# astomodynamics/cddp-cpp

Hardware: AMD Instinct MI355X
Metric: trajectories_per_sec (higher is better)
Workload: dtype f64

## Files before the change

### cddp-cpp_amd/csrc/capi.hip

```cpp
#include <algorithm>
#include <chrono>
#include <cmath>
#include <cstdarg>
#include <cstddef>
#include <cstdio>
#include <cstdlib>
#include <cstring>
#include <string>
#include <vector>
#include <map>

#include "launch.hpp"
#include "plant.hpp"
#include "io_kernels.hpp"
#include "sens_kernels.hpp"
#include "score_kernels.hpp"
#include "mppi_kernels.hpp"

static int ladder_strictly_decreasing(const double *a, int n) {
  for (int i = 1; i < n; ++i) if (!(a[i] < a[i - 1])) return 0;
  return n > 0 ? 1 : 0;
}

using namespace cddp_dev;
// ... 850 lines not shown
  HIPCHK(hipStreamSynchronize(h->stream));
  return 0;
}

static int in_set_terminal(Inner *h, const double *S_T, const double *Y_T, const double *Lambda_T) {
  if (!h) return fail(-1, "null handle");
  if (h->P.n_term <= 0) return fail(-1, "cddp_hip_set_terminal: the problem has no terminal constraints");
  if (!h->has_state) return fail(-1, "cddp_hip_set_terminal needs an initialised handle");
  HIPCHK(hipSetDevice(h->device));
  const DevBuf &d = h->d;
  struct { const double *host; double *dev; int n; } items[] = {{S_T, d.ST, h->P.mT}, {Y_T, d.YT, h->P.mT}, {Lambda_T, d.LamT, h->P.pT}};
  for (auto &it : items) {
    if (!it.host || it.n <= 0) continue;
    std::vector<double> buf((size_t)it.n * d.Bp, 0.0);
    for (int b = 0; b < d.B; ++b) for (int i = 0; i < it.n; ++i) buf[(size_t)i * d.Bp + b] = it.host[(size_t)b * it.n + i];
    HIPCHK(hipMemcpyAsync(it.dev, buf.data(), buf.size() * sizeof(double), hipMemcpyHostToDevice, h->stream));
    HIPCHK(hipStreamSynchronize(h->stream));
  }
  return 0;
}

static int in_backward(Inner *h, int32_t *ok) {
  if (!h) return fail(-1, "null handle");
  HIPCHK(hipSetDevice(h->device));
  if (!h->initialized) { int rc = in_initialize(h); if (rc) return rc; }
  h->ks->derivs(h->d, h->route, 1, h->stream);
  h->ks->backward(h->d, h->route, h->P.solver, 1, 0, h->stream);
  HIPCHK(hipGetLastError());
  if (ok) HIPCHK(hipMemcpyAsync(ok, h->d.bwd_ok, sizeof(int) * h->d.B, hipMemcpyDeviceToHost, h->stream));
  HIPCHK(hipStreamSynchronize(h->stream));
  return 0;
}

static int in_forward(Inner *h, const double *alphas, int n_alphas, cddp_hip_trial *trials) {
  if (!h || !alphas || !trials) return fail(-1, "null argument");
  if (n_alphas <= 0 || n_alphas > h->d.n_alphas) return fail(-1, "n_alphas must be in [1, %d] (the handle's ladder size)", h->d.n_alphas);
  HIPCHK(hipSetDevice(h->device));
  ProblemDev tmp = h->P;
  for (int i = 0; i < n_alphas; ++i) tmp.alphas[i] = alphas[i];
  HIPCHK(hipMemcpyAsync(h->dP, &tmp, sizeof(ProblemDev), hipMemcpyHostToDevice, h->stream));
  DevBuf dcall = h->d;
  dcall.ladder_sorted = ladder_strictly_decreasing(tmp.alphas, h->d.n_alphas);
  h->ks->forward(dcall, h->route, h->P.solver, 0, n_alphas, PH_FWD1, 1, 0, h->stream, 0, 0);
  h->ks->costate(dcall, h->route, h->P.solver, 0, n_alphas, PH_FWD1, 1, 0, h->stream);
  HIPCHK(hipGetLastError());
  const DevBuf &d = h->d;
  const size_t n = (size_t)n_alphas * d.Bp;
  std::vector<double> c(n), mf(n), th(n), ipr(n), ic(n), ap(n), ad(n);
  std::vector<int> su(n);
  HIPCHK(hipMemcpyAsync(c.data(), d.t_cost, n * 8, hipMemcpyDeviceToHost, h->stream));
  HIPCHK(hipMemcpyAsync(mf.data(), d.t_merit, n * 8, hipMemcpyDeviceToHost, h->stream));
  HIPCHK(hipMemcpyAsync(th.data(), d.t_theta, n * 8, hipMemcpyDeviceToHost, h->stream));
  HIPCHK(hipMemcpyAsync(ipr.data(), d.t_inf_pr, n * 8, hipMemcpyDeviceToHost, h->stream));
  HIPCHK(hipMemcpyAsync(ic.data(), d.t_inf_comp, n * 8, hipMemcpyDeviceToHost, h->stream));
  HIPCHK(hipMemcpyAsync(ap.data(), d.t_apr, n * 8, hipMemcpyDeviceToHost, h->stream));
  HIPCHK(hipMemcpyAsync(ad.data(), d.t_adu, n * 8, hipMemcpyDeviceToHost, h->stream));
  HIPCHK(hipMemcpyAsync(su.data(), d.t_success, n * 4, hipMemcpyDeviceToHost, h->stream));
  HIPCHK(hipMemcpyAsync(h->dP, &h->P, sizeof(ProblemDev), hipMemcpyHostToDevice, h->stream));
  HIPCHK(hipStreamSynchronize(h->stream));
  for (int b = 0; b < d.B; ++b)
    for (int a = 0; a < n_alphas; ++a) {
      cddp_hip_trial &t = trials[(size_t)b * n_alphas + a];
      const size_t i = (size_t)a * d.Bp + b;
      t.alpha = alphas[a]; t.alpha_pr = ap[i]; t.alpha_du = ad[i]; t.cost = c[i]; t.merit_function = mf[i];
      t.theta = th[i]; t.inf_pr = ipr[i]; t.inf_comp = ic[i]; t.success = (su[i] == 1) ? 1 : 0; t._pad = 0;
    }
  return 0;
}

struct SolveRun {
  Inner *h = nullptr;
  bool want_stats = false;
  int conc = 1;
  int detail = -1;
  std::vector<int> ev_slot;
  size_t ev_used = 0;
// ... 28 lines not shown
    const bool want = detail == CDDP_HIP_TIMING_ALL ||
                      (detail == CDDP_HIP_TIMING_ROLLOUT && (point == 1 || point == 2 || (two_stage_marks && (point == 3 || point == 4)))) ||
                      (detail == CDDP_HIP_TIMING_SWEEP && (point == 0 || point == 1));
    if (!want) return;
    if (ev_used == h->ev_pool.size()) {
      hipEvent_t e;
      if ((h->knob->event_fence ? hipEventCreate(&e) : hipEventCreateWithFlags(&e, hipEventDisableSystemFence)) != hipSuccess) return;
      h->ev_pool.push_back(e);
    }
    const size_t slot = (size_t)6 * (size_t)(outer - 1) + (size_t)point;
    if (ev_slot.size() <= slot) ev_slot.resize(slot + 1, -1);
    hipEventRecord(h->ev_pool[ev_used], h->stream);
    ev_slot[slot] = (int)ev_used++;
  }

  void adapt_ladder(int window_iters) {
    if (pinned) return;
    long total = 0;
    std::vector<long> hd(na + 1);
    for (int a = 0; a <= na; ++a) { hd[a] = (long)hist_now[a] - (long)hist_prev[a]; total += hd[a]; }
    hist_prev = hist_now;
    if (total <= 0) return;
    const long allow = std::max(1L, (long)window_iters / 4);
    int kq = na;
    long tail = hd[na];
    for (int k = na - 1; k >= 1; --k) {
      tail += hd[k];
      if (tail <= allow) kq = k; else break;
    }
    if (kq >= na - 1) {
      if (waves_all <= 2048) { one_stage = true; }
      else { one_stage = false; k1 = k_cap2; }
    } else {
      one_stage = false; k1 = std::max(1, std::min(kq + h->knob->ls_margin, k_cap));
      if (waves_all <= 2048 && (long)k1 * per_alpha_waves > two_stage_max_waves) one_stage = true;
      const long small_cap = (h->P.solver == CDDP_HIP_SOLVER_LOGDDP || h->P.solver == CDDP_HIP_SOLVER_MSIPDDP) ? 2048 : 1024;
      if (waves_all <= small_cap && h->P.nx <= 8 && h->knob->ls_small_frac * k1 > na) one_stage = true;
    }
    if (h->knob->debug_ladder) {
      std::fprintf(stderr, "[ladder] it=%d total=%ld kq=%d -> %s k1=%d hist:", outer, total, kq, one_stage ? "one" : "two", k1);
      for (int a = 0; a <= na; ++a) std::fprintf(stderr, " %ld", hd[a]);
      std::fprintf(stderr, "\n");
    }
  }

  int begin(Inner *h_, bool stats_, int conc_) {
    h = h_; want_stats = stats_; conc = std::max(1, conc_);
    const ProblemDev &P = h->P;
    const DevBuf &d = h->d;
    hipStream_t s = h->stream;
    const KernelSet *ks = h->ks;
    max_it = P.opt.max_iterations;
    first_rule = (P.ls_rule == CDDP_HIP_LS_FIRST_SUCCESS);
    na = d.n_alphas;
    use_graph = h->knob->graph;
    if (use_graph && conc > 1) {
      static bool said = false;
      if (!said) { said = true; std::fprintf(stderr, "[cddp_hip] CDDP_HIP_GRAPH=1: graph replay does not keep the CU-masked streams' partition; the tile groups share the whole chip\n"); }
    }
    detail = (want_stats && !use_graph) ? h->timing_detail : -1;
    if (!h->ev_begin) { HIPCHK(hipEventCreate(&h->ev_begin)); HIPCHK(hipEventCreate(&h->ev_end)); }
    if (!h->ev_poll) { HIPCHK(hipEventCreateWithFlags(&h->ev_poll, hipEventDisableTiming)); HIPCHK(hipEventCreateWithFlags(&h->ev_poll2, hipEventDisableTiming)); }
    poll_evs[0] = h->ev_poll; poll_evs[1] = h->ev_poll2;
    win_enq = win_dig = 0; ran_ahead = false;
    if (!h->h_poll) HIPCHK(hipHostMalloc((void **)&h->h_poll, sizeof(int) * 2 * kPollWords));
    HIPCHK(hipMemsetAsync(h->d_launched, 0, sizeof(unsigned long long) * kLsGran, s));
    HIPCHK(hipEventRecord(h->ev_begin, s));
    pre_has_state = h->has_state;
    shadow = !force_sync && shadow_eligible(h, conc) && max_it > 0;
    redo_needed = false;
    inkernel = shadow && P.ls_rule == CDDP_HIP_LS_FIRST_SUCCESS && h->knob->ls_inkernel &&
               (h->route.rollout == Route::kPair || h->route.rollout == Route::kTwoConsumers);
    poll_us = h->knob->ls_poll_us >= 0 ? h->knob->ls_poll_us : kLsPollUs;
    h->ls_counts[0] = h->ls_counts[1] = h->ls_counts[2] = 0;
    if (inkernel && !h->h_ls) HIPCHK(hipHostMalloc((void **)&h->h_ls, sizeof(unsigned long long) * kLsGran));
    h->last_shadow = shadow; h->ever_solved = true;
    if (shadow) HIPCHK(hipMemsetAsync(h->d.cs_bad, 0, sizeof(int), s));
// ... 23 lines not shown
  void enqueue_iteration(int last) {
    const ProblemDev &P = h->P;
    if (shadow) {
      DevBuf &hd = h->d;
      hd.Vx_prev = hd.Vx; hd.Vxx_prev = hd.Vxx;
      std::swap(hd.Vx, hd.Vx2); std::swap(hd.Vxx, hd.Vxx2);
      hd.cs_vsel ^= 1;
    }
    DevBuf dsh = h->d;
    if (shadow) {
      h->cs_epoch += 2;
      dsh.cs_mode = 1; dsh.cs_stamp = h->cs_epoch + 1; dsh.cs_want = dsh.cs_stamp - 2;
      dsh.cs_fail_stamp = h->knob->fail_shadow > 0 ? stamp0 + 2 * h->knob->fail_shadow + 1 : 0;
    }
    const DevBuf &d = dsh;
    hipStream_t s = h->stream;
    const KernelSet *ks = h->ks;
    const Route &r = h->route;
    hipStream_t sf = h->cu.fwd ? h->cu.fwd : s;
    auto to_fwd = [&](int k) { if (sf != s) { order_check(hipEventRecord(h->cu.ev[k], s)); order_check(hipStreamWaitEvent(sf, h->cu.ev[k], 0)); } };
    auto from_fwd = [&](int k) { if (sf != s) { order_check(hipEventRecord(h->cu.ev[k], sf)); order_check(hipStreamWaitEvent(s, h->cu.ev[k], 0)); } };
    const bool split = !one_stage && inkernel;
    two_stage_marks = !one_stage && !split;
    mark(0);
    ks->derivs(d, r, 0, s);
    tl_sweep_hop = h->cu.sweep ? &h->cu.hop : nullptr;
    if (shadow && outer > 1) { dsh.cs_extra = ks->shadow_extra(d, r); ks->backward(dsh, r, P.solver, 0, 1, s); dsh.cs_extra = 0; }
    else ks->backward(d, r, P.solver, 0, 1, s);
    tl_sweep_hop = nullptr;
    mark(1);
    to_fwd(0);
    if (fwd_wait) hipStreamWaitEvent(sf, fwd_wait, 0);
    if (one_stage || split) {
      ks->forward(d, r, P.solver, 0, na, PH_FWD1, 0, first_rule ? 1 : 0, sf, split ? k1 : 0, poll_us);
      if (fwd_done) hipEventRecord(fwd_done, sf);
      from_fwd(1);
      mark(2);
      if (!shadow) ks->costate(d, r, P.solver, 0, na, PH_FWD1, 0, first_rule ? 1 : 2, s);
      ks->update(d, r, 1, na, last, 1, s);
      mark(3);
      launches += shadow ? 3 : 4;
    } else {
      ks->forward(d, r, P.solver, 0, k1, PH_FWD1, 0, 1, sf, 0, 0);
      from_fwd(1);
      mark(2);
      if (!shadow) ks->costate(d, r, P.solver, 0, k1, PH_FWD1, 0, 1, s);
      if (shadow) {
        DevBuf d1 = dsh;
        d1.cs_stamp = h->cs_epoch;
        ks->update(d1, r, 1, k1, last, 0, s);
        d1.cs_want = d1.cs_stamp; d1.Vx_prev = d1.Vx; d1.Vxx_prev = d1.Vxx;
        ks->shadow_flush(d1, nullptr, s);
      } else
      ks->update(d, r, 1, k1, last, 0, s);
      mark(3);
      to_fwd(2);
      ks->forward(d, r, P.solver, k1, na - k1, PH_FWD2, 0, 1, sf, 0, 0);
      if (fwd_done) hipEventRecord(fwd_done, sf);
      from_fwd(3);
      mark(4);
      if (!shadow) ks->costate(d, r, P.solver, k1, na - k1, PH_FWD2, 0, 1, s);
      ks->update(d, r, 2, na, last, 1, s);
      mark(5);
      launches += shadow ? 5 : 6;
    }
  }
  bool polled_iteration(int i) const { return i % h->knob->poll_every == 0 || i == max_it || (i <= 2 && !pinned); }

  int advance_graph() {
    const hipStream_t s = h->stream;
    int w = 0;
    while (it + w < max_it) { ++w; if (polled_iteration(it + w)) break; }
    if (w == 0) { done = true; return 0; }
    const int last = (it + w == max_it) ? 1 : 0;
    const unsigned long long key = ((unsigned long long)(one_stage ? 0 : k1) << 16) | ((unsigned long long)w << 4) | (unsigned long long)last;
    auto f = h->graphs.find(key);
    if (f == h->graphs.end()) {
      hipGraph_t g = nullptr; hipGraphExec_t ge = nullptr;
      const int launches0 = launches;
      HIPCHK(hipStreamBeginCapture(s, hipStreamCaptureModeThreadLocal));
      for (int j = 1; j <= w; ++j) enqueue_iteration((j == w) ? last : 0);
      HIPCHK(hipStreamEndCapture(s, &g));
      HIPCHK(hipGraphInstantiate(&ge, g, nullptr, nullptr, 0));
      hipGraphDestroy(g);
      launches = launches0;
      f = h->graphs.emplace(key, ge).first;
    }
    { const int l0 = launches; for (int j = 0; j < w; ++j) launches += one_stage ? 4 : 6; (void)l0; }
    HIPCHK(hipGraphLaunch(f->second, s));
    it += w; outer += w;
// ... 1530 lines not shown
```

### cddp-cpp_amd/csrc/kernels_lean.hpp

```cpp
#pragma once
#include "kernels.hpp"

namespace cddp_dev {

#define GI(t, E, e) (((((size_t)(t)) * (size_t)d.NB + (size_t)(b >> 6)) * (E) + (e)) * 64 + (size_t)(b & 63))

template <class Model, class Cons>
struct CstLayout {
  static constexpr int NX = Model::NX, NU = Model::NU;
  static constexpr int CX = 0, CU = CX + NX, WQYU = CU + NU, QYUSIR = WQYU + NU * NU, IPR = QYUSIR + NU, ICOMP = IPR + 1;
  static constexpr int WQYX = ICOMP + 1, QYXSIR = WQYX + NU * NX, WXQYX = QYXSIR + NX;
  static constexpr int SIZE = Cons::HAS_X ? (WXQYX + NX * NX) : WQYX;
};

template <class Model, class Cons, bool WITH_DERIVS>
DEV void condense_eval(const ProblemDev *__restrict__ P, const double *__restrict__ xrt, const int t, const double *x, const double *u,
                       const double *y, const double *s, const double *g, const double mu, double *A, double *Bq, double *c,
                       double *ys_out = nullptr) {
  constexpr int NX = Model::NX, NU = Model::NU, M = Cons::M;
  typedef Objective<NX, NU> Obj;
  typedef CstLayout<Model, Cons> L;
  const double s_floor = dmax(mu * 1e-3, kEpsSlack);
  double Qyx[M * NX], Qyu[M * NU];
  if constexpr (WITH_DERIVS) {
// ... 580 lines not shown
template <class Model>
__global__ __launch_bounds__(64) void k_costate_flush(DevBuf d) {
  costate_shadow_item<Model::NX>(d, blockIdx.x * 64 + threadIdx.x, blockIdx.y);
}

template <int NX>
__global__ __launch_bounds__(64) void k_value_merge(DevBuf d) {
  const int b = blockIdx.x * 64 + threadIdx.x, t = blockIdx.y;
  if (b >= d.B || d.cs_vbuf[b] == d.cs_vsel) return;
  double vx[NX], vxx[NX * NX];
  ld<NX>(d.Vx2 + GI(t, NX, 0), kLS, vx);
  ld<NX * NX>(d.Vxx2 + GI(t, NX * NX, 0), kLS, vxx);
  st<NX>(d.Vx + GI(t, NX, 0), kLS, vx);
  st<NX * NX>(d.Vxx + GI(t, NX * NX, 0), kLS, vxx);
}
#ifdef CDDP_K4_TIMING
__device__ unsigned long long g_k4_times[16384 * 4];
#define K4_TIME_BEGIN const unsigned long long k4_t0 = wall_clock64();
#define K4_TIME_END(role, steps) do { if (lane == 0) { const size_t k4_i = ((size_t)blockIdx.y * gridDim.x + blockIdx.x) * 4 + (role) * 2; \
    g_k4_times[k4_i] = wall_clock64() - k4_t0; g_k4_times[k4_i + 1] = (unsigned long long)(steps); } } while (0)
#else
#define K4_TIME_BEGIN
#define K4_TIME_END(role, steps)
#endif
template <int NX, int NU> struct RollIn { double x[NX], u[NU]; };
template <int NX> struct RollOut { double xn[NX]; };
template <class Model>
__device__ __attribute__((noinline)) RollOut<Model::NX> roll_step_checked(int integrator, double dt, const double *mp, RollIn<Model::NX, Model::NU> in) {
  RollOut<Model::NX> o;
  Stepper<Model>::step(integrator, dt, mp, in.x, in.u, o.xn);
  return o;
}

template <class Model, class Cons, bool TERM = false, int NC = 1>
__global__ __launch_bounds__(64 * (1 + NC)) void k_forward_ipddp_pc(DevBuf d, const ProblemDev *__restrict__ Pk, const double *__restrict__ xrt,
                                                                    int a0, int phase_req, int force, int k1, int poll_us) {
  constexpr int NX = Model::NX, NU = Model::NU, M = Cons::M;
  typedef Objective<NX, NU> Obj;
  static_assert(M > 0, "two-role rollout is for path-constrained problems");
  constexpr int RW = 2 * NX + NU;
  constexpr int kRing = RW <= 10 ? 8 : (RW <= 20 ? 4 : 2);
  __shared__ double s_ring[kRing * RW * 64];
  static_assert(NC == 1 || NC == 2, "one or two consumer waves");
  __shared__ int s_prod;
  __shared__ int s_consv[2];
  [[maybe_unused]] __shared__ int s_abort;
  [[maybe_unused]] __shared__ int s_done1;
  constexpr int kL2 = NC > 1 ? 64 : 1;
  [[maybe_unused]] __shared__ int s_pfail[kL2], s_palive[kL2];
  [[maybe_unused]] __shared__ double s_pmax[4 * kL2];
  [[maybe_unused]] __shared__ double s_prun[kL2];
  __shared__ unsigned s_need[2];
  __shared__ int s_pstat[64];
  __shared__ double s_pcost[64];
  __shared__ double s_xN[TERM ? NX * 64 : 1];
  __shared__ double s_obj[Obj::kStage];
  const int lane = threadIdx.x & 63;
  K4_TIME_BEGIN
  const int wave = __builtin_amdgcn_readfirstlane((int)threadIdx.x) >> 6;
  const bool producer = wave == 0;
  [[maybe_unused]] const int ci = NC > 1 ? wave - 1 : 0;
  int *const s_cons = &s_consv[0];
  const int b = blockIdx.x * 64 + lane;
  const int a = a0 + blockIdx.y;
  const ProblemDev *__restrict__ P = Pk;
  const cddp_hip_options &o = P->opt;
  const int N = d.N;
  bool active = (b < d.B) && (force || d.phase[b] == phase_req);
  if (__builtin_amdgcn_ballot_w64(active) == 0ull) return;
// ... 23 lines not shown
    if (lane == 0) {
      s_need[0] = (unsigned)need; s_need[1] = (unsigned)(need >> 32);
      atomicAdd(d.launched + (need != 0ull ? kLsRan : kLsRet), 1ull);
      if (gave_up) atomicAdd(d.launched + kLsGiveUp, 1ull);
    }
  }
  __syncthreads();
  if (stage2) {
    const unsigned n0 = __builtin_amdgcn_readfirstlane(s_need[0]), n1 = __builtin_amdgcn_readfirstlane(s_need[1]);
    if ((n0 | n1) == 0u) return;
    active = active && ((((lane < 32 ? n0 : n1) >> (lane & 31)) & 1u) != 0u);
  }
  auto publish_mask = [&](const bool ok) {
    if (k1 > 0 && a < k1) {
      const unsigned long long m = __builtin_amdgcn_ballot_w64(ok);
      if (lane < 2)
        __hip_atomic_store(d.launched + kLsGran + ((size_t)blockIdx.x * CDDP_HIP_MAX_ALPHAS + a) * 2 + lane,
                           ((unsigned long long)kLsTag << 32) | (unsigned long long)(unsigned)(m >> (32 * lane)), __ATOMIC_RELAXED, __HIP_MEMORY_SCOPE_AGENT);
    }
  };
  const int bb = (b < d.B) ? b : 0;
  const int cur = (b < d.B) ? d.cur[b] : 0;
  const int slot = trial_slot(cur, a);
  const double *Xc = d.X + (size_t)cur * d.planeX;
  const double alpha = P->alphas[a];
  const double a_pr = dmin(alpha, d.apr_max[bb]);
  auto wait_ge = [&](int *ctr, int need) -> int {
    int v;
    while ((v = __hip_atomic_load(ctr, __ATOMIC_RELAXED, __HIP_MEMORY_SCOPE_WORKGROUP)) < need) __builtin_amdgcn_s_sleep(1);
    asm volatile("" ::: "memory");
    return v;
  };
  const int kAbort = 2 * N + kRing;

  if (producer) {
    double *Xn = d.X + (size_t)slot * d.planeX;
    double *Un = d.U + (size_t)slot * d.planeU;
    const double *Uc = d.U + (size_t)cur * d.planeU;
    bool alive = active;
    double x[NX];
    ld<NX>(Xc + GI(0, NX, 0), kLS, x);
    st<NX>(Xn + GI(0, NX, 0), kLS, x);
    struct StepIn { double xo[NX], uo[NU], kk[NU], KK[NU * NX]; };
    const size_t rs1 = (size_t)d.NB * 64;
    const double *ld_X = Xc + GI(0, NX, 0), *ld_U = Uc + GI(0, NU, 0), *ld_k = d.k + GI(0, NU, 0), *ld_K = d.K + GI(0, NU * NX, 0);
    double *st_U = Un + GI(0, NU, 0), *st_X = Xn + GI(1, NX, 0);
    auto load_step = [&](int tt, StepIn &r) {
      ld<NX>(Xc + GI(tt, NX, 0), kLS, r.xo);
      ld<NU>(Uc + GI(tt, NU, 0), kLS, r.uo);
      ld<NU>(d.k + GI(tt, NU, 0), kLS, r.kk);
      ld<NU * NX>(d.K + GI(tt, NU * NX, 0), kLS, r.KK);
    };
    auto load_row = [&](StepIn &r) {
      ld<NX>(ld_X, kLS, r.xo);
      ld<NU>(ld_U, kLS, r.uo);
      ld<NU>(ld_k, kLS, r.kk);
      ld<NU * NX>(ld_K, kLS, r.KK);
    };
    auto advance_ld = [&](const int t) {
      const size_t s = t + 1 < N ? rs1 : 0;
      ld_X += s * NX; ld_U += s * NU; ld_k += s * NU; ld_K += s * (NU * NX);
    };
    DynCtx dc;
    dc.load(P->integrator, P->dt, P->mp);
    [[maybe_unused]] typename Obj::Ctx oc_p;
    [[maybe_unused]] double run_cost_p = 0.0;
    if constexpr (NC > 1) Obj::load_staged(P, oc_p, s_obj);
    auto prime = [&]() {
      double z[NX];
#pragma unroll
      for (int i = 0; i < NX; ++i) z[i] = 0.0;
      st<NU>(Un + GI(0, NU, 0), kLS, z);
      st<NX>(Xn + GI(1, NX, 0), kLS, z);
    };
    constexpr bool kPing = sizeof(StepIn) <= 40 * sizeof(double);
    constexpr bool kEarly = !kPing && sizeof(StepIn) <= 96 * sizeof(double);
    constexpr bool kChunkP = !kPing && !kEarly;
    struct PChunk { double K[NX], uo, kk; };
    auto load_pchunk = [&](int tt, const int i, PChunk &c) {
      ld<NX>(d.K + GI(tt, NU * NX, i * NX), kLS, c.K);
      c.uo = Uc[GI(tt, NU, i)]; c.kk = d.k[GI(tt, NU, i)];
    };
    PChunk pk0, pk1;
    double xo_c[NX];
    constexpr bool kFlagged = kPing && HasTrigPolicy<Model>::value && NC == 1;
    auto step = [&](auto integ, const int t, StepIn &cs, StepIn &nxt) {
      constexpr int INTEG = decltype(integ)::value;
      if constexpr (kPing) {
        advance_ld(t);
        load_row(nxt);
      }
      PIPELINE_FENCE();
      double dx[NX], u[NU], xn[NX];
      bool finite = true;
      if constexpr (kChunkP) {
#pragma unroll
        for (int i = 0; i < NX; ++i) dx[i] = x[i] - xo_c[i];
#pragma unroll
        for (int i = 0; i < NU; ++i) {
          if (i + 1 < NU) { if ((i & 1) == 0) load_pchunk(t, i + 1, pk1); else load_pchunk(t, i + 1, pk0); }
          __builtin_amdgcn_sched_barrier(0);
          const PChunk &c = (i & 1) == 0 ? pk0 : pk1;
          double s1 = 0.0;
#pragma unroll
          for (int j = 0; j < NX; ++j) s1 += c.K[j] * dx[j];
          u[i] = (c.uo + a_pr * c.kk) + s1;
          finite = finite && dfinite(u[i]);
          __builtin_amdgcn_sched_barrier(0);
        }
      } else {
#pragma unroll
      for (int i = 0; i < NX; ++i) dx[i] = x[i] - cs.xo[i];
#pragma unroll
      for (int i = 0; i < NU; ++i) {
        double s1 = 0.0;
#pragma unroll
        for (int j = 0; j < NX; ++j) s1 += cs.KK[i * NX + j] * dx[j];
        u[i] = (cs.uo[i] + a_pr * cs.kk[i]) + s1;
        finite = finite && dfinite(u[i]);
      }
      }
// ... 22 lines not shown
        load_pchunk(tn, 0, pk0);
        PIPELINE_FENCE();
      }
      [[maybe_unused]] bool redo = false;
      if constexpr (kPing) roll_step<Model, INTEG, kFlagged>(dc, x, u, xn, &redo);
      else Stepper<Model>::step(dc, x, u, xn);
      if constexpr (kFlagged) {
        if (__builtin_expect(__builtin_amdgcn_ballot_w64(redo) != 0ull, 0)) {
          RollIn<NX, NU> in;
#pragma unroll
          for (int i = 0; i < NX; ++i) in.x[i] = x[i];
#pragma unroll
          for (int i = 0; i < NU; ++i) in.u[i] = u[i];
          const RollOut<NX> o = roll_step_checked<Model>(dc.integrator, dc.dt, P->mp, in);
#pragma unroll
          for (int i = 0; i < NX; ++i) xn[i] = o.xn[i];
        }
      }
#pragma unroll
      for (int i = 0; i < NX; ++i) finite = finite && dfinite(xn[i]);
      if (alive && !finite) { s_pstat[lane] = t; alive = false; }
      if constexpr (kPing) {
        st<NU>(st_U, kLS, u);
        st<NX>(st_X, kLS, xn);
        st_U += rs1 * NU; st_X += rs1 * NX;
      } else {
        st<NU>(Un + GI(t, NU, 0), kLS, u);
        st<NX>(Xn + GI(t + 1, NX, 0), kLS, xn);
      }
      if (alive) {
#pragma unroll
        for (int i = 0; i < NX; ++i) x[i] = xn[i];
      }
    };
    int t = 0;
    auto walk = [&](auto integ) {
      if constexpr (kPing) {
        StepIn R[2];
        load_row(R[0]);
        prime();
        for (; t + 1 < N; t += 2) {
#pragma unroll
          for (int j = 0; j <= 1; ++j) step(integ, t + j, R[j], R[(j + 1) % 2]);
          if (__builtin_amdgcn_ballot_w64(alive) == 0ull) { t = N; break; }
        }
#pragma unroll
        for (int j = 0; j <= 1; ++j) if (t + j < N) step(integ, t + j, R[j], R[(j + 1) % 2]);
      } else {
        StepIn ra;
        if constexpr (kChunkP) { ld<NX>(Xc + GI(0, NX, 0), kLS, xo_c); load_pchunk(0, 0, pk0); } else load_step(0, ra);
        prime();
        for (; t < N; ++t) {
          step(integ, t, ra, ra);
          if (__builtin_amdgcn_ballot_w64(alive) == 0ull) break;
        }
      }
    };
    if constexpr (Model::kDiscrete || !kPing) walk(std::integral_constant<int, CDDP_HIP_RK4>());
    else switch (dc.integrator) {
      case CDDP_HIP_EULER: walk(std::integral_constant<int, CDDP_HIP_EULER>()); break;
      case CDDP_HIP_HEUN: walk(std::integral_constant<int, CDDP_HIP_HEUN>()); break;
      case CDDP_HIP_RK3: walk(std::integral_constant<int, CDDP_HIP_RK3>()); break;
      default: walk(std::integral_constant<int, CDDP_HIP_RK4>()); break;
    }
    if (alive) s_pcost[lane] = Obj::terminal_cost(P, x);
    if constexpr (NC > 1) s_prun[lane] = run_cost_p;
// ... 40 lines not shown
    ld<M>(d.ys + GI(tt, M, 0), kLS, r.ys);
  };
  typename Cons::Ctx cc;
  Cons::load(P, cc);
  typename Obj::Ctx oc;
  Obj::load_staged(P, oc, s_obj);
  auto prime = [&]() {
    double z[M];
#pragma unroll
    for (int i = 0; i < M; ++i) z[i] = 0.0;
    const int tp = (NC > 1 && ci < N) ? ci : 0;
    st<M>(Sn + GI(tp, M, 0), kLS, z);
    st<M>(Yn + GI(tp, M, 0), kLS, z);
    st<M>(Gn + GI(tp, M, 0), kLS, z);
    double *ev = d.ev + GI((size_t)a * N + tp, 2 * Cons::NSEG, 0);
#pragma unroll
    for (int c = 0; c < Cons::NSEG; ++c) { if (c > 0 || NC > 1) ev[(size_t)(Cons::NSEG + c) * kLS] = 0.0; ev[(size_t)c * kLS] = 0.0; }
  };
  constexpr bool kPing = sizeof(StepIn) <= 40 * sizeof(double);
  constexpr bool kEarly = !kPing && sizeof(StepIn) <= 96 * sizeof(double);
  constexpr bool kChunk = !kPing && !kEarly && UDiag<Cons>::value && M == 2 * NU;
  struct Chunk { double K[NX], s[2], y[2], ksv[2], ky[2], ys[2]; };
  auto load_chunk = [&](int tt, const int i, Chunk &c) {
    ld<NX>(d.K + GI(tt, NU * NX, i * NX), kLS, c.K);
#pragma unroll
    for (int h = 0; h < 2; ++h) {
      const int r = i + h * NU;
      c.s[h] = Sc[GI(tt, M, r)]; c.y[h] = Yc[GI(tt, M, r)];
      c.ksv[h] = d.ks[GI(tt, M, r)]; c.ky[h] = d.ky[GI(tt, M, r)]; c.ys[h] = d.ys[GI(tt, M, r)];
    }
  };
  Chunk ck0, ck1;
  auto step = [&](const int t, StepIn &cs, StepIn &nxt) {
    if constexpr (kPing) {
      const int tn = t + NC < N ? t + NC : N - 1;
      load_step(tn, nxt);
    } else if constexpr (!kEarly && !kChunk) load_step(t, cs);
    PIPELINE_FENCE();
    if (seen_prod < t + 1) seen_prod = __builtin_amdgcn_readfirstlane(wait_ge(&s_prod, t + 1));
    double rx[NX], dx[NX], u[NU];
    {
      const double *rs = s_ring + (size_t)(t % kRing) * RW * 64 + lane;
#pragma unroll
      for (int i = 0; i < NX; ++i) { rx[i] = rs[i * 64]; dx[i] = rs[(NX + i) * 64]; }
#pragma unroll
      for (int i = 0; i < NU; ++i) u[i] = rs[(2 * NX + i) * 64];
      RING_FENCE();
      __hip_atomic_store(&s_consv[ci], t + 1, __ATOMIC_RELAXED, __HIP_MEMORY_SCOPE_WORKGROUP);
    }
    if (alive && s_pstat[lane] <= t) { alive = false; fail_t = t; }
    double sn[M], yn[M];
    bool feas = true;
    if constexpr (kChunk) {
      auto rows = [&](const int i, const Chunk &c) {
#pragma unroll
        for (int h = 0; h < 2; ++h) {
          const int r = i + h * NU;
          const double gv = UDiag<Cons>::val(cc, r);
          double Ksr[NX], Kyr[NX];
#pragma unroll
          for (int cix = 0; cix < NX; ++cix) {
            const double s2 = 0.0 + gv * c.K[cix];
            const double inner = 0.0 + s2;
            Kyr[cix] = dmin(dmax(c.ys[h] * inner, -kMaxBarrierRatio), kMaxBarrierRatio);
            Ksr[cix] = (-0.0) - s2;
          }
          sn[r] = affine_2r<NX>(c.s[h], a_pr, c.ksv[h], Ksr, dx);
// ... 54 lines not shown
      if (!dfinite(sn[r]) || !dfinite(yn[r])) feas = false;
    }
    }
    fail_t = (alive && !feas) ? t : fail_t;
    if (!feas) alive = false;
    st<M>(Sn + GI(t, M, 0), kLS, sn);
    st<M>(Yn + GI(t, M, 0), kLS, yn);
    if constexpr (kEarly) {
      load_step(t + 1 < N ? t + 1 : t, cs);
      PIPELINE_FENCE();
    }
    double g[M];
    Cons::template eval<NX, NU>(cc, rx, u, g);
    if constexpr (NC == 1) run_cost += Obj::running_cost(oc, xrt, t, rx, u);
    st<M>(Gn + GI(t, M, 0), kLS, g);
    double *ev = d.ev + GI((size_t)a * N + t, 2 * Cons::NSEG, 0);
#pragma unroll
    for (int c = 0; c < Cons::NSEG; ++c) {
      const int off = Cons::seg_off(c), dim = Cons::seg_dim(c);
      double n1 = 0.0, ninf = 0.0, ls = 0.0;
      for (int i = 0; i < dim; ++i) {
        const double r = g[off + i] + sn[off + i];
        n1 += l2norm ? r * r : fabs(r);
        ninf = dmax(ninf, fabs(r));
        const double ysp = yn[off + i] * sn[off + i];
        ev_icomp = dmax(ev_icomp, fabs(ysp - mu));
        ys_lo = dmin(ys_lo, ysp); ys_hi = dmax(ys_hi, ysp);
        ls += solver_log(dmax(sn[off + i], kEpsSlack));
      }
      ev_max = dmax(ev_max, ninf);
      if (c == 0 && NC == 1) ev_total0 += n1; else ev[(size_t)(Cons::NSEG + c) * kLS] = n1;
      ev[(size_t)c * kLS] = ls;
    }
  };
  StepIn ra;
  if constexpr (NC > 1) {
    static_assert(NC == 1 || kPing, "two consumers: ping-pong records with one step of look-ahead only");
    StepIn R0, R1;
    load_step(ci < N ? ci : N - 1, R0);
    prime();
    auto stop_at = [&](int tt) { return tt > __hip_atomic_load(&s_abort, __ATOMIC_RELAXED, __HIP_MEMORY_SCOPE_WORKGROUP); };
    int t = ci, last = -1;
    bool stopped = false;
    for (; t + NC < N; t += 2 * NC) {
      if (stop_at(t)) { stopped = true; break; }
      step(t, R0, R1); last = t;
      if (stop_at(t + NC)) { stopped = true; break; }
      step(t + NC, R1, R0); last = t + NC;
      if (__builtin_amdgcn_ballot_w64(alive) == 0ull) {
        __hip_atomic_fetch_min(&s_abort, last, __ATOMIC_RELAXED, __HIP_MEMORY_SCOPE_WORKGROUP);
        stopped = true; break;
      }
    }
    if (!stopped && t < N && !stop_at(t)) step(t, R0, R1);
    const bool aborted = __hip_atomic_load(&s_abort, __ATOMIC_RELAXED, __HIP_MEMORY_SCOPE_WORKGROUP) != 0x7fffffff;
    if (aborted) __hip_atomic_store(&s_consv[ci], kAbort, __ATOMIC_RELAXED, __HIP_MEMORY_SCOPE_WORKGROUP);
    if (ci == 1) {
      s_pfail[lane] = fail_t; s_palive[lane] = alive ? 1 : 0;
      s_pmax[lane] = ev_max; s_pmax[64 + lane] = ev_icomp; s_pmax[128 + lane] = ys_lo; s_pmax[192 + lane] = ys_hi;
      __builtin_amdgcn_fence(__ATOMIC_RELEASE, "workgroup");
      __hip_atomic_store(&s_done1, 1, __ATOMIC_RELAXED, __HIP_MEMORY_SCOPE_WORKGROUP);
      return;
    }
    wait_ge(&s_done1, 1);
    __builtin_amdgcn_fence(__ATOMIC_ACQUIRE, "workgroup");
    fail_t = s_pfail[lane] < fail_t ? s_pfail[lane] : fail_t;
// ... 101 lines not shown
        dp += lam * h;
      }
    }
    mer += dp;
  }
  const double th = l2norm ? sqrt(total) : total;
  const double theta_new = dmax(th, ev_max), phi_new = mer, ipr = ev_max, icomp = ev_icomp;
  if (!dfinite(phi_new) || !dfinite(theta_new) || !dfinite(ipr) || !dfinite(icomp)) return;
  bool accept = false;
  {
    const double expected_improvement = a_pr * d.dV0[b];
    const int fn = d.filt_n[b];
    const double cv_old = (fn == 0) ? 0.0 : d.filt[(size_t)(kFilterCap + fn - 1) * d.Bp + b];
    const double high_ref = (fn == 0) ? d.filter_theta[b] : cv_old;
    const double merit_old = d.merit[b];
    if (theta_new > o.filter_max_violation_threshold) {
      if (theta_new < (1 - o.filter_violation_acceptance_threshold) * high_ref) accept = true;
    } else if (dmax(theta_new, cv_old) < o.filter_min_violation_for_armijo_check && expected_improvement < 0) {
      if (phi_new < merit_old + o.filter_armijo_constant * expected_improvement) accept = true;
    } else {
      if (phi_new < merit_old - o.filter_merit_acceptance_threshold * theta_new ||
          theta_new < (1 - o.filter_violation_acceptance_threshold) * cv_old) accept = true;
    }
  }
  d.t_cost[ti] = cost_new; d.t_merit[ti] = phi_new; d.t_theta[ti] = theta_new;
  d.t_inf_pr[ti] = ipr; d.t_inf_comp[ti] = icomp;
  d.t_ysmin[ti] = ys_lo; d.t_ysmax[ti] = ys_hi;
  d.t_success[ti] = accept ? 1 : 0;
  flagged = accept;
  }();
  publish_mask(flagged);
}

#undef GI
}
```

### cddp-cpp_amd/csrc/knobs.hpp

```cpp
#pragma once
#include <climits>
#include <cstdlib>
#include <cstring>
#include <string>

namespace cddp_dev {

inline char env_first(const char *name) { const char *e = std::getenv(name); return e ? e[0] : 0; }
inline bool env_is(const char *name, const char *v) { const char *e = std::getenv(name); return e && !std::strcmp(e, v); }
inline int env_num(const char *name, int dflt, int lo, int hi) { const char *e = std::getenv(name); const int n = e ? std::atoi(e) : dflt; return (n >= lo && n <= hi) ? n : dflt; }
inline long env_long(const char *name, long dflt) { const char *e = std::getenv(name); return e ? std::atol(e) : dflt; }
inline std::string env_str(const char *name) { const char *e = std::getenv(name); return e ? e : ""; }

struct Knobs {
  enum Sweep { kSweepCoop, kSweepLane, kSweepElem, kSweepMfma };
  int sweep = env_is("CDDP_HIP_SWEEP", "lane") ? kSweepLane : env_is("CDDP_HIP_SWEEP", "elem") ? kSweepElem : env_is("CDDP_HIP_SWEEP", "mfma") ? kSweepMfma : kSweepCoop;
  bool t4 = env_first("CDDP_HIP_T4") != '0';
  int sweep_roles = env_num("CDDP_HIP_SWEEP_ROLES", 1, 0, 2);
  bool coop_h2 = env_first("CDDP_HIP_COOP_H") == '2';
  bool coop_w1 = env_first("CDDP_HIP_COOP_W") == '1';
  int k4_na = env_num("CDDP_HIP_K4_NA", 1, 1, 3);
  bool k4_consumers2 = env_first("CDDP_HIP_K4_CONSUMERS") == '2';
  bool ms_lane_rollout = env_is("CDDP_HIP_MS_ROLLOUT", "lane");
  bool lg_lane_rollout = env_is("CDDP_HIP_LG_ROLLOUT", "lane");
  bool graph = env_first("CDDP_HIP_GRAPH") == '1';
  char ls_stages = env_first("CDDP_HIP_LS_STAGES");
  int ls_first = env_num("CDDP_HIP_LS_FIRST", 0, INT_MIN, INT_MAX);
  long ls_two_max_waves = env_long("CDDP_HIP_LS_TWO_MAX_WAVES", 768);
  int ls_small_frac = env_num("CDDP_HIP_LS_SMALL_FRAC", 3, 1, INT_MAX);
  int ls_margin = env_num("CDDP_HIP_LS_MARGIN", 1, 0, 8);
  bool ls_inkernel = env_first("CDDP_HIP_LS_INKERNEL") != '0';
  int ls_poll_us = env_num("CDDP_HIP_TEST_LS_POLL_US", -1, 0, INT_MAX);
  int run_ahead = env_num("CDDP_HIP_RUNAHEAD", 1, 0, 16);
  int poll_every = env_num("CDDP_HIP_POLL_EVERY", 4, 1, INT_MAX);
  bool event_fence = env_first("CDDP_HIP_EVENT_FENCE") == '1';
  bool debug_ladder = std::getenv("CDDP_HIP_DEBUG_LADDER") != nullptr;
  int groups = env_num("CDDP_HIP_GROUPS", 0, INT_MIN, INT_MAX);
  bool chunking = env_num("CDDP_HIP_CHUNK", 1, INT_MIN, INT_MAX) > 0;
  int chunk = env_num("CDDP_HIP_CHUNK", 0, 1, INT_MAX);
  int partition = env_num("CDDP_HIP_PARTITION", 0, 1, 16);
  bool cumask_set = std::getenv("CDDP_HIP_CUMASK") != nullptr;
  std::string cumask = env_str("CDDP_HIP_CUMASK");
  bool pingpong = env_first("CDDP_HIP_PINGPONG") == '1';
  bool xcd_map = env_first("CDDP_HIP_XCD_MAP") != '0';
  int fail_costate = env_num("CDDP_HIP_TEST_FAIL_COSTATE", 0, INT_MIN, INT_MAX);
  enum Costate { kCostateAuto, kCostateSync, kCostateShadow };
  int costate = env_is("CDDP_HIP_COSTATE", "sync") ? kCostateSync : env_is("CDDP_HIP_COSTATE", "shadow") ? kCostateShadow : kCostateAuto;
  int fail_shadow = env_num("CDDP_HIP_TEST_FAIL_SHADOW", 0, 1, INT_MAX);
};

}
```

### cddp-cpp_amd/csrc/launch.hpp

```cpp
#pragma once
#include <algorithm>
#include <vector>
#include "knobs.hpp"
#include "kernels_te.hpp"
#include "kernels_pcm.hpp"
#include "kernels_elem.hpp"
#include "kernels_mfma.hpp"
#include "kernels_logddp.hpp"
#include "kernels_msipddp.hpp"

namespace cddp_dev {

struct SweepHop { hipStream_t s; hipEvent_t ev_in, ev_out; };
inline thread_local const SweepHop *tl_sweep_hop = nullptr;
inline thread_local hipError_t tl_order_error = hipSuccess;
inline void order_check(hipError_t e) { if (e != hipSuccess && tl_order_error == hipSuccess) tl_order_error = e; }
inline hipStream_t sweep_hop_in(hipStream_t s) {
  const SweepHop *h = tl_sweep_hop;
  if (!h || h->s == s) return s;
  order_check(hipEventRecord(h->ev_in, s));
  order_check(hipStreamWaitEvent(h->s, h->ev_in, 0));
  return h->s;
}
inline void sweep_hop_out(hipStream_t s) {
  const SweepHop *h = tl_sweep_hop;
  if (!h || h->s == s) return;
  order_check(hipEventRecord(h->ev_out, h->s));
  order_check(hipStreamWaitEvent(s, h->ev_out, 0));
}

struct Route {
  enum Sweep { kCoop, kLane, kElem, kMfma, kRowSplit, kOneWave };
  enum Rollout { kPair, kGroup2, kGroup3, kTwoConsumers, kLaneRollout };
  int sweep = kCoop;
  int roles_nh = 0;
  bool ms_split = false;
  int rollout = kPair;
  int t4 = 0;
};

struct KernelSet {
  int model, nx, nu, m;
  int cst_size;
  int te_rec_size, te_group;
  const char *name;
  bool (*matches)(const ProblemDev &);
  Route (*route)(const DevBuf &, int solver, const Knobs &);
  void (*derivs)(const DevBuf &, const Route &, int force, hipStream_t);
  void (*backward)(const DevBuf &, const Route &, int solver, int force, int count_iter, hipStream_t);
  void (*forward)(const DevBuf &, const Route &, int solver, int a0, int na, int phase_req, int force, int first_only, hipStream_t, int k1, int poll_us);
  void (*costate)(const DevBuf &, const Route &, int solver, int a0, int na, int phase_req, int force, int first_only, hipStream_t);
  void (*update)(const DevBuf &, const Route &, int stage, int n1, int is_last, int do_count, hipStream_t);
  void (*init)(const DevBuf &, int mode, hipStream_t);
  void (*stage)(const DevBuf &, int copy_xu, int ipddp, hipStream_t);
  int (*sweep_blocks)(const DevBuf &);
  int (*shadow_extra)(const DevBuf &, const Route &);
  void (*shadow_flush)(const DevBuf &, const DevBuf *, hipStream_t);
  bool logddp_ddp;
  bool has_msipddp;
  bool has_logddp;
  int ms_cst_size;
};

template <class Model, class Cons> struct PcTwoConsumers { static constexpr bool value = false; };
template <class Cons> struct PcTwoConsumers<UnicycleModel, Cons> {
  static constexpr int kRec = 5 * Cons::M + UnicycleModel::NU * UnicycleModel::NX + (Cons::HAS_X ? UnicycleModel::NX : 1) + (Cons::NEEDS_U ? UnicycleModel::NU : 1);
  static constexpr bool value = Cons::M >= 4 && kRec > 16 && kRec <= 40;
};

template <class Model, class Cons, bool TERM = false>
struct Launcher {
  static bool matches(const ProblemDev &P) {
    return P.model == Model::ID && P.nx == Model::NX && P.nu == Model::NU && Cons::matches(P) && (TERM ? P.n_term > 0 : P.n_term == 0);
  }
  static constexpr bool kLean = !TERM && Cons::M > 0;
  static constexpr int cst_size() { if constexpr (kLean) return CstLayout<Model, Cons>::SIZE; else return 0; }
  static constexpr bool kTeCoop = TERM && !Cons::HAS_X;
  static constexpr int te_rec_size() { if constexpr (kTeCoop) return TeCfg<Model, Cons>::REC; else return 0; }
  static constexpr int kLogMaxNx = 16;
  static constexpr bool kLog = !TERM && Model::NX <= kLogMaxNx;
  static constexpr int kMsMaxNx = 13;
  static constexpr bool kMs = !TERM && Model::NX <= kMsMaxNx && (Cons::M == 0 || Model::NU == 1 || Model::NX == Model::NU);
  static constexpr int ms_cst_size() { if constexpr (kMs && Cons::M > 0) return MsCst<Model, Cons>::SIZE; else return 0; }
  static dim3 gridB(const DevBuf &d) { return dim3((d.B + 63) / 64); }
  template <int RB> static constexpr bool roles_fit() {
    if constexpr (!kLean || Model::NX > 8) return false;
    else return (size_t)RoleCfg<Model, Cons, RB>::RING * 8 + (size_t)CoopCfg<Model>::TPW * CoopCfg<Model>::STRIDE * 8 <= (size_t)72 * 1024;
  }
  static constexpr bool kRoles = roles_fit<2>();
  static Route route(const DevBuf &d, int solver, const Knobs &k) {
    Route r;
    const bool lane = k.sweep == Knobs::kSweepLane || (d.ddp && solver != CDDP_HIP_SOLVER_CLDDP);
    r.sweep = lane ? Route::kLane : Route::kCoop;
    r.ms_split = d.ms && d.cst && !lane;
    if (solver == CDDP_HIP_SOLVER_IPDDP && !lane) {
      if constexpr (kLean && Model::NX > 8) {
        if (Model::NX <= 15 && Model::NU <= 8 && k.sweep == Knobs::kSweepMfma) r.sweep = Route::kMfma;
        else if (k.coop_h2) r.sweep = Route::kRowSplit;
        else if (Cons::HAS_X || k.coop_w1) r.sweep = Route::kOneWave;
      } else if constexpr (kLean) {
        if (Model::NX <= 4 && Model::NU <= 2 && k.sweep == Knobs::kSweepElem) r.sweep = Route::kElem;
// ... 112 lines not shown
              else if constexpr (roles_fit<3>()) hipLaunchKernelGGL((k_backward_ipddp_coop<Model, Cons, 2, 3>), gridC, dim3(192), 0, ss, d, d.P, d.xref_traj, force, count_iter);
              else hipLaunchKernelGGL((k_backward_ipddp_coop<Model, Cons, 2, 2>), gridC, dim3(192), 0, ss, d, d.P, d.xref_traj, force, count_iter);
            }
            sweep_hop_out(s);
          }
        } else {
          hipLaunchKernelGGL((k_backward_ipddp_coop<Model, Cons>), gridC, dim3(64), 0, sweep_hop_in(s), d, d.P, d.xref_traj, force, count_iter);
          sweep_hop_out(s);
        }
      }
      if constexpr (kRoles) { if (r.roles_nh > 0) return; }
      hipLaunchKernelGGL((k_post<Model, Cons>), dim3((d.B + 63) / 64, d.N), dim3(64), 0, s, d, d.P, force);
    } else if constexpr (!TERM && Cons::M == 0) {
      if (lane_sweep)
        hipLaunchKernelGGL((k_backward_ipddp<Model, Cons, TERM>), gridB(d), dim3(64), 0, s, d, d.P, d.xref_traj, force, count_iter);
      else {
        hipLaunchKernelGGL((k_backward_coop_plain<Model, false>), gridC, dim3(64), 0, sweep_hop_in(s), d, d.P, d.xref_traj, force, count_iter);
        sweep_hop_out(s);
      }
    } else {
      if constexpr (kTeCoop) {
        if (r.sweep == Route::kCoop) {
          hipLaunchKernelGGL((k_backward_te_coop<Model, Cons>), gridC, dim3(64), 0, sweep_hop_in(s), d, d.P, d.xref_traj, force, count_iter);
          sweep_hop_out(s);
          const int tiles = (d.B + 63) / 64;
          int tstep = (int)(((long long)tiles * d.N) / 1024); if (tstep < 1) tstep = 1; if (tstep > 16) tstep = 16;
          hipLaunchKernelGGL((k_te_post<Model, Cons>), dim3(tiles, (d.N + tstep - 1) / tstep), dim3(64), 0, s, d, d.P, force, tstep);
          return;
        }
      }
      hipLaunchKernelGGL((k_backward_ipddp<Model, Cons, TERM>), gridB(d), dim3(64), 0, s, d, d.P, d.xref_traj, force, count_iter);
    }
  }
  static void forward(const DevBuf &d, const Route &r, int solver, int a0, int na, int phase_req, int force, int first_only, hipStream_t s, int k1 = 0, int poll_us = 0) {
    if (na <= 0) return;
    const dim3 grid((d.B + 63) / 64, na);
    if (solver == CDDP_HIP_SOLVER_LOGDDP) {
      if constexpr (kLog) {
        if (r.rollout == Route::kLaneRollout) hipLaunchKernelGGL((k_forward_logddp<Model, Cons>), grid, dim3(64), 0, s, d, d.P, d.xref_traj, a0, 0, phase_req, force);
        else hipLaunchKernelGGL((k_forward_logddp_pc<Model, Cons>), grid, dim3(128), 0, s, d, d.P, d.xref_traj, a0, phase_req, force);
      }
      return;
    }
    if (solver == CDDP_HIP_SOLVER_MSIPDDP) {
      if constexpr (kMs) {
        if (r.rollout == Route::kLaneRollout || !d.ladder_sorted) hipLaunchKernelGGL((k_forward_msipddp<Model, Cons>), grid, dim3(64), 0, s, d, d.P, d.xref_traj, a0, 0, phase_req, force);
        else hipLaunchKernelGGL((k_forward_msipddp_pc<Model, Cons>), grid, dim3(128), 0, s, d, d.P, d.xref_traj, a0, phase_req, force);
      }
      return;
    }
    if (solver == CDDP_HIP_SOLVER_CLDDP)
      hipLaunchKernelGGL((k_forward_clddp<Model>), grid, dim3(64), 0, s, d, d.P, d.xref_traj, a0, 0, phase_req, force);
    else
    {
      if constexpr (kLean) {
        if constexpr (PcmTraits<Model, Cons>::kOk) {
          if (r.rollout == Route::kGroup3) { hipLaunchKernelGGL((k_forward_ipddp_pcm<Model, Cons, 3>), dim3((d.B + 63) / 64, (na + 2) / 3), dim3(256), 0, s, d, d.P, d.xref_traj, a0, na, phase_req, force); return; }
          if (r.rollout == Route::kGroup2) { hipLaunchKernelGGL((k_forward_ipddp_pcm<Model, Cons, 2>), dim3((d.B + 63) / 64, (na + 1) / 2), dim3(192), 0, s, d, d.P, d.xref_traj, a0, na, phase_req, force); return; }
        }
        if constexpr (PcTwoConsumers<Model, Cons>::value) {
          if (r.rollout == Route::kTwoConsumers) { hipLaunchKernelGGL((k_forward_ipddp_pc<Model, Cons, false, 2>), grid, dim3(192), 0, s, d, d.P, d.xref_traj, a0, phase_req, force, k1, poll_us); return; }
        }
        hipLaunchKernelGGL((k_forward_ipddp_pc<Model, Cons>), grid, dim3(128), 0, s, d, d.P, d.xref_traj, a0, phase_req, force, k1, poll_us);
      } else {
        if constexpr (kTeCoop && Cons::M > 0) {
          if (r.sweep == Route::kCoop) {
            hipLaunchKernelGGL((k_forward_ipddp_pc<Model, Cons, true>), grid, dim3(128), 0, s, d, d.P, d.xref_traj, a0, phase_req, force, 0, 0);
            return;
          }
        }
        hipLaunchKernelGGL((k_forward_ipddp<Model, Cons, TERM>), grid, dim3(64), 0, s, d, d.P, d.xref_traj, a0, 0, phase_req, force);
      }
    }
    (void)first_only;
  }
  static void costate(const DevBuf &d, const Route &r, int solver, int a0, int na, int phase_req, int force, int first_only, hipStream_t s) {
    if (solver == CDDP_HIP_SOLVER_MSIPDDP) {
      if constexpr (kMs) {
        if (na <= 0 || r.rollout == Route::kLaneRollout || !d.ladder_sorted) return;
        if (!force && first_only == 2) hipLaunchKernelGGL((k_pick_candidate<0>), dim3((d.B + 63) / 64), dim3(64), 0, s, d, a0, na, phase_req, force);
        hipLaunchKernelGGL((k_rows_msipddp<Model, Cons>), dim3((d.B + 63) / 64, d.N), dim3(64), 0, s, d, d.P, a0, na, phase_req, force, first_only);
      }
      return;
    }
    if (na <= 0 || solver == CDDP_HIP_SOLVER_CLDDP || solver == CDDP_HIP_SOLVER_LOGDDP) return;
    if (!force && first_only == 2) hipLaunchKernelGGL((k_pick_candidate<0>), dim3((d.B + 63) / 64), dim3(64), 0, s, d, a0, na, phase_req, force);
    if constexpr (Model::NX > 8) {
      if (!force && first_only != 0) {
        hipLaunchKernelGGL((k_costate_one<Model>), dim3((d.B + 63) / 64, d.N + 1), dim3(64), 0, s, d, a0, na, phase_req, first_only);
        return;
      }
    }
    hipLaunchKernelGGL((k_costate<Model>), dim3((d.B + 63) / 64, d.N + 1), dim3(64), 0, s, d, a0, na, phase_req, force, force ? 0 : first_only);
  }
// ... 71 lines not shown
```

Measured before the change: 111,400.

## Time-slice wave priority in paired forward rollout via clock-based setprio

Adds a sliced variant of the producer/consumer IPDDP forward rollout kernel. At each step it reads the wall clock and toggles s_setprio, so that early and late workgroups alternate high priority in time slices when the grid oversubscribes the SIMDs. The aim is to stop starvation and tail imbalance among oversubscribed waves. The default line-search margin also becomes 0 when the in-kernel split is used, down from 1. The slicing adds clock reads and priority switches on every step and applies only to the cartpole and unicycle models on the pair route.

Result: faster. 116,800 (median of 6 runs) (+4.8%).

```diff
diff --git a/cddp-cpp_amd/csrc/capi.hip b/cddp-cpp_amd/csrc/capi.hip
--- a/cddp-cpp_amd/csrc/capi.hip
+++ b/cddp-cpp_amd/csrc/capi.hip
@@ -906,6 +906,22 @@
   return 0;
 }
 
+constexpr int kK4SliceUs = 2;
+static RollSlice roll_slice_for(const Inner *h, int conc, int n_run) {
+  RollSlice sl;
+  const Knobs &k = *h->knob;
+  if (k.k4_slice_us == 0 || h->P.solver != CDDP_HIP_SOLVER_IPDDP || h->route.rollout != Route::kPair) return sl;
+  const long simds = std::max(4L, (long)device_cu_count(h->device) * 4 / std::max(1, conc)), waves_per_wg = 2;
+  sl.late_from = (int)(simds / waves_per_wg);
+  const bool forced = k.k4_slice_us > 0;
+  if (!forced && (long)((h->d.B + 63) / 64) * n_run * waves_per_wg <= simds) return sl;
+  if (k.k4_late_prio) { sl.ticks = kSliceFixedLate; return sl; }
+  const long want = 100L * (forced ? k.k4_slice_us : kK4SliceUs);
+  sl.ticks = 1ull;
+  while ((long)sl.ticks * 4 < want * 3) sl.ticks <<= 1;
+  return sl;
+}
+
 static int in_forward(Inner *h, const double *alphas, int n_alphas, cddp_hip_trial *trials) {
   if (!h || !alphas || !trials) return fail(-1, "null argument");
   if (n_alphas <= 0 || n_alphas > h->d.n_alphas) return fail(-1, "n_alphas must be in [1, %d] (the handle's ladder size)", h->d.n_alphas);
@@ -915,7 +931,7 @@
   HIPCHK(hipMemcpyAsync(h->dP, &tmp, sizeof(ProblemDev), hipMemcpyHostToDevice, h->stream));
   DevBuf dcall = h->d;
   dcall.ladder_sorted = ladder_strictly_decreasing(tmp.alphas, h->d.n_alphas);
-  h->ks->forward(dcall, h->route, h->P.solver, 0, n_alphas, PH_FWD1, 1, 0, h->stream, 0, 0);
+  h->ks->forward(dcall, h->route, h->P.solver, 0, n_alphas, PH_FWD1, 1, 0, h->stream, 0, 0, roll_slice_for(h, 1, n_alphas));
   h->ks->costate(dcall, h->route, h->P.solver, 0, n_alphas, PH_FWD1, 1, 0, h->stream);
   HIPCHK(hipGetLastError());
   const DevBuf &d = h->d;
@@ -1010,7 +1026,8 @@
       if (waves_all <= 2048) { one_stage = true; }
       else { one_stage = false; k1 = k_cap2; }
     } else {
-      one_stage = false; k1 = std::max(1, std::min(kq + h->knob->ls_margin, k_cap));
+      const int margin = h->knob->ls_margin >= 0 ? h->knob->ls_margin : (inkernel ? 0 : 1);
+      one_stage = false; k1 = std::max(1, std::min(kq + margin, k_cap));
       if (waves_all <= 2048 && (long)k1 * per_alpha_waves > two_stage_max_waves) one_stage = true;
       const long small_cap = (h->P.solver == CDDP_HIP_SOLVER_LOGDDP || h->P.solver == CDDP_HIP_SOLVER_MSIPDDP) ? 2048 : 1024;
       if (waves_all <= small_cap && h->P.nx <= 8 && h->knob->ls_small_frac * k1 > na) one_stage = true;
@@ -1021,6 +1038,8 @@
       std::fprintf(stderr, "\n");
     }
   }
+
+  RollSlice roll_slice(int n_run) const { return roll_slice_for(h, conc, n_run); }
 
   int begin(Inner *h_, bool stats_, int conc_) {
     h = h_; want_stats = stats_; conc = std::max(1, conc_);
@@ -1110,7 +1129,7 @@
     to_fwd(0);
     if (fwd_wait) hipStreamWaitEvent(sf, fwd_wait, 0);
     if (one_stage || split) {
-      ks->forward(d, r, P.solver, 0, na, PH_FWD1, 0, first_rule ? 1 : 0, sf, split ? k1 : 0, poll_us);
+      ks->forward(d, r, P.solver, 0, na, PH_FWD1, 0, first_rule ? 1 : 0, sf, split ? k1 : 0, poll_us, roll_slice(split ? k1 : na));
       if (fwd_done) hipEventRecord(fwd_done, sf);
       from_fwd(1);
       mark(2);
@@ -1119,7 +1138,7 @@
       mark(3);
       launches += shadow ? 3 : 4;
     } else {
-      ks->forward(d, r, P.solver, 0, k1, PH_FWD1, 0, 1, sf, 0, 0);
+      ks->forward(d, r, P.solver, 0, k1, PH_FWD1, 0, 1, sf, 0, 0, roll_slice(k1));
       from_fwd(1);
       mark(2);
       if (!shadow) ks->costate(d, r, P.solver, 0, k1, PH_FWD1, 0, 1, s);
@@ -1133,7 +1152,7 @@
       ks->update(d, r, 1, k1, last, 0, s);
       mark(3);
       to_fwd(2);
-      ks->forward(d, r, P.solver, k1, na - k1, PH_FWD2, 0, 1, sf, 0, 0);
+      ks->forward(d, r, P.solver, k1, na - k1, PH_FWD2, 0, 1, sf, 0, 0, RollSlice());
       if (fwd_done) hipEventRecord(fwd_done, sf);
       from_fwd(3);
       mark(4);
diff --git a/cddp-cpp_amd/csrc/kernels_lean.hpp b/cddp-cpp_amd/csrc/kernels_lean.hpp
--- a/cddp-cpp_amd/csrc/kernels_lean.hpp
+++ b/cddp-cpp_amd/csrc/kernels_lean.hpp
@@ -636,9 +636,10 @@
   return o;
 }
 
-template <class Model, class Cons, bool TERM = false, int NC = 1>
-__global__ __launch_bounds__(64 * (1 + NC)) void k_forward_ipddp_pc(DevBuf d, const ProblemDev *__restrict__ Pk, const double *__restrict__ xrt,
-                                                                    int a0, int phase_req, int force, int k1, int poll_us) {
+template <class Model, class Cons, bool TERM, int NC, bool SL>
+__device__ __forceinline__ void forward_ipddp_pc(const DevBuf &d, const ProblemDev *__restrict__ Pk, const double *__restrict__ xrt,
+                                                 int a0, int phase_req, int force, int k1, int poll_us,
+                                                 [[maybe_unused]] const unsigned long long slice_ticks, [[maybe_unused]] const int late_from) {
   constexpr int NX = Model::NX, NU = Model::NU, M = Cons::M;
   typedef Objective<NX, NU> Obj;
   static_assert(M > 0, "two-role rollout is for path-constrained problems");
@@ -728,6 +729,11 @@
     return v;
   };
   const int kAbort = 2 * N + kRing;
+  constexpr bool kSlice = SL && NC == 1;
+  [[maybe_unused]] const unsigned long long slice_late = (int)(blockIdx.y * gridDim.x + blockIdx.x) >= late_from ? slice_ticks : 0ull;
+  [[maybe_unused]] auto slice_prio = [&](const unsigned long long clk) {
+    if (((clk & slice_ticks) ^ slice_late) != 0ull) __builtin_amdgcn_s_setprio(3); else __builtin_amdgcn_s_setprio(0);
+  };
 
   if (producer) {
     double *Xn = d.X + (size_t)slot * d.planeX;
@@ -782,7 +788,9 @@
     constexpr bool kFlagged = kPing && HasTrigPolicy<Model>::value && NC == 1;
     auto step = [&](auto integ, const int t, StepIn &cs, StepIn &nxt) {
       constexpr int INTEG = decltype(integ)::value;
+      [[maybe_unused]] unsigned long long clk = 0ull;
       if constexpr (kPing) {
+        if constexpr (kSlice) clk = wall_clock64();
         advance_ld(t);
         load_row(nxt);
       }
@@ -871,6 +879,7 @@
 #pragma unroll
         for (int i = 0; i < NX; ++i) x[i] = xn[i];
       }
+      if constexpr (kPing && kSlice) slice_prio(clk);
     };
     int t = 0;
     auto walk = [&](auto integ) {
@@ -977,7 +986,9 @@
   };
   Chunk ck0, ck1;
   auto step = [&](const int t, StepIn &cs, StepIn &nxt) {
+    [[maybe_unused]] unsigned long long clk = 0ull;
     if constexpr (kPing) {
+      if constexpr (kSlice) clk = wall_clock64();
       const int tn = t + NC < N ? t + NC : N - 1;
       load_step(tn, nxt);
     } else if constexpr (!kEarly && !kChunk) load_step(t, cs);
@@ -1098,6 +1109,7 @@
       if (c == 0 && NC == 1) ev_total0 += n1; else ev[(size_t)(Cons::NSEG + c) * kLS] = n1;
       ev[(size_t)c * kLS] = ls;
     }
+    if constexpr (kPing && kSlice) slice_prio(clk);
   };
   StepIn ra;
   if constexpr (NC > 1) {
@@ -1265,5 +1277,17 @@
   publish_mask(flagged);
 }
 
+template <class Model, class Cons, bool TERM = false, int NC = 1>
+__global__ __launch_bounds__(64 * (1 + NC)) void k_forward_ipddp_pc(DevBuf d, const ProblemDev *__restrict__ Pk, const double *__restrict__ xrt,
+                                                                    int a0, int phase_req, int force, int k1, int poll_us) {
+  forward_ipddp_pc<Model, Cons, TERM, NC, false>(d, Pk, xrt, a0, phase_req, force, k1, poll_us, 0ull, 0);
+}
+template <class Model, class Cons>
+__global__ __launch_bounds__(128) void k_forward_ipddp_pc_sl(DevBuf d, const ProblemDev *__restrict__ Pk, const double *__restrict__ xrt,
+                                                             int a0, int phase_req, int force, int k1, int poll_us,
+                                                             unsigned long long slice_ticks, int late_from) {
+  forward_ipddp_pc<Model, Cons, false, 1, true>(d, Pk, xrt, a0, phase_req, force, k1, poll_us, slice_ticks, late_from);
+}
+
 #undef GI
 }
diff --git a/cddp-cpp_amd/csrc/knobs.hpp b/cddp-cpp_amd/csrc/knobs.hpp
--- a/cddp-cpp_amd/csrc/knobs.hpp
+++ b/cddp-cpp_amd/csrc/knobs.hpp
@@ -21,6 +21,8 @@
   bool coop_w1 = env_first("CDDP_HIP_COOP_W") == '1';
   int k4_na = env_num("CDDP_HIP_K4_NA", 1, 1, 3);
   bool k4_consumers2 = env_first("CDDP_HIP_K4_CONSUMERS") == '2';
+  int k4_slice_us = env_num("CDDP_HIP_K4_SLICE_US", -1, 0, 10000);
+  bool k4_late_prio = env_first("CDDP_HIP_K4_LATE_PRIO") == '1';
   bool ms_lane_rollout = env_is("CDDP_HIP_MS_ROLLOUT", "lane");
   bool lg_lane_rollout = env_is("CDDP_HIP_LG_ROLLOUT", "lane");
   bool graph = env_first("CDDP_HIP_GRAPH") == '1';
@@ -28,7 +30,7 @@
   int ls_first = env_num("CDDP_HIP_LS_FIRST", 0, INT_MIN, INT_MAX);
   long ls_two_max_waves = env_long("CDDP_HIP_LS_TWO_MAX_WAVES", 768);
   int ls_small_frac = env_num("CDDP_HIP_LS_SMALL_FRAC", 3, 1, INT_MAX);
-  int ls_margin = env_num("CDDP_HIP_LS_MARGIN", 1, 0, 8);
+  int ls_margin = env_num("CDDP_HIP_LS_MARGIN", -1, 0, 8);
   bool ls_inkernel = env_first("CDDP_HIP_LS_INKERNEL") != '0';
   int ls_poll_us = env_num("CDDP_HIP_TEST_LS_POLL_US", -1, 0, INT_MAX);
   int run_ahead = env_num("CDDP_HIP_RUNAHEAD", 1, 0, 16);
diff --git a/cddp-cpp_amd/csrc/launch.hpp b/cddp-cpp_amd/csrc/launch.hpp
--- a/cddp-cpp_amd/csrc/launch.hpp
+++ b/cddp-cpp_amd/csrc/launch.hpp
@@ -39,6 +39,9 @@
   int t4 = 0;
 };
 
+struct RollSlice { unsigned long long ticks = 0; int late_from = 0; };
+constexpr unsigned long long kSliceFixedLate = 1ull << 62;
+
 struct KernelSet {
   int model, nx, nu, m;
   int cst_size;
@@ -48,7 +51,7 @@
   Route (*route)(const DevBuf &, int solver, const Knobs &);
   void (*derivs)(const DevBuf &, const Route &, int force, hipStream_t);
   void (*backward)(const DevBuf &, const Route &, int solver, int force, int count_iter, hipStream_t);
-  void (*forward)(const DevBuf &, const Route &, int solver, int a0, int na, int phase_req, int force, int first_only, hipStream_t, int k1, int poll_us);
+  void (*forward)(const DevBuf &, const Route &, int solver, int a0, int na, int phase_req, int force, int first_only, hipStream_t, int k1, int poll_us, RollSlice);
   void (*costate)(const DevBuf &, const Route &, int solver, int a0, int na, int phase_req, int force, int first_only, hipStream_t);
   void (*update)(const DevBuf &, const Route &, int stage, int n1, int is_last, int do_count, hipStream_t);
   void (*init)(const DevBuf &, int mode, hipStream_t);
@@ -67,6 +70,10 @@
   static constexpr int kRec = 5 * Cons::M + UnicycleModel::NU * UnicycleModel::NX + (Cons::HAS_X ? UnicycleModel::NX : 1) + (Cons::NEEDS_U ? UnicycleModel::NU : 1);
   static constexpr bool value = Cons::M >= 4 && kRec > 16 && kRec <= 40;
 };
+
+template <class Model, class Cons> struct PcSlice { static constexpr bool value = false; };
+template <class Cons> struct PcSlice<CartPoleModel, Cons> { static constexpr bool value = Cons::M > 0; };
+template <class Cons> struct PcSlice<UnicycleModel, Cons> { static constexpr bool value = Cons::M > 0; };
 
 template <class Model, class Cons, bool TERM = false>
 struct Launcher {
@@ -245,7 +252,7 @@
       hipLaunchKernelGGL((k_backward_ipddp<Model, Cons, TERM>), gridB(d), dim3(64), 0, s, d, d.P, d.xref_traj, force, count_iter);
     }
   }
-  static void forward(const DevBuf &d, const Route &r, int solver, int a0, int na, int phase_req, int force, int first_only, hipStream_t s, int k1 = 0, int poll_us = 0) {
+  static void forward(const DevBuf &d, const Route &r, int solver, int a0, int na, int phase_req, int force, int first_only, hipStream_t s, int k1 = 0, int poll_us = 0, RollSlice sl = RollSlice()) {
     if (na <= 0) return;
     const dim3 grid((d.B + 63) / 64, na);
     if (solver == CDDP_HIP_SOLVER_LOGDDP) {
@@ -273,6 +280,9 @@
         }
         if constexpr (PcTwoConsumers<Model, Cons>::value) {
           if (r.rollout == Route::kTwoConsumers) { hipLaunchKernelGGL((k_forward_ipddp_pc<Model, Cons, false, 2>), grid, dim3(192), 0, s, d, d.P, d.xref_traj, a0, phase_req, force, k1, poll_us); return; }
+        }
+        if constexpr (PcSlice<Model, Cons>::value) {
+          if (sl.ticks != 0ull) { hipLaunchKernelGGL((k_forward_ipddp_pc_sl<Model, Cons>), grid, dim3(128), 0, s, d, d.P, d.xref_traj, a0, phase_req, force, k1, poll_us, sl.ticks, sl.late_from); return; }
         }
         hipLaunchKernelGGL((k_forward_ipddp_pc<Model, Cons>), grid, dim3(128), 0, s, d, d.P, d.xref_traj, a0, phase_req, force, k1, poll_us);
       } else {
```
